# shrubb/latent-pose-reenactment

Hardware: AMD Instinct MI355X
Metric: train-step images/sec at 256x256 bs=8 (higher is better)
Workload: dtype mixed 16-bit MFMA operands, fp32 accumulate, fp32 activations / weights / optimizer state; 1 GPU; default.yaml meta-training step (configs[2]): ResNeXt50 identity encoder over 8 frames + MobileNetV2 pose encoder (both trained, forward + backward on hand-written gfx950 kernels), G, D with the 98000x512 label embedding, VGG19/VGGFace/featmat/adversarial/dis_embed/dice criterions, Adam, EMA; image_size=256, per_gpu_batch=8, global_batch=8, parallelism=dp1, precision_mode=default assignment (LP_PREC=f16), padding=zero, launch_mode=hipgraph

## Files before the change

### include/lp_hip.h

```cpp
#ifndef LP_HIP_H
#define LP_HIP_H
#include <stdint.h>
#ifdef __cplusplus
extern "C" {
#endif

#define LP_OK 0
#define LP_ERR_ARG (-1)
#define LP_ERR_UNSUPPORTED (-2)
#define LP_ERR_HIP (-3)

#define LP_PREC_BF16 0
#define LP_PREC_BF16X3 1
#define LP_PREC_F16 2

const char* lp_last_error(void);
int lp_abi_version(void);

int lp_pack_weights(const float* w, uint16_t* hi, uint16_t* lo, int Cout, int Cin, int T, int RowsP, int ColsP, int mode, int f16,
                    void* stream);
int lp_pack_desc_bytes(void);
int lp_pack_weights_batch(const void* table, int num_entries, long long total_chunks, void* stream);
int lp_pack_pair_desc_bytes(void);
int lp_pack_weights_pairs(const void* table, int num_entries, long long total_tiles, void* stream);

int lp_act_pack(const float* x, const float* scale, const float* shift, int pro, uint16_t* hi, uint16_t* lo,
                int N, int HW, int C, int prec, const float* in_scale, const float* amax_part, int amax_count, int amax_stride,
                float* scale_out, void* stream);
int lp_amax_blocks(void);
int lp_amax_slots(void);
int lp_amax_slot_stride(void);
int lp_amax_partial(const float* x, long long numel, float* part, void* stream);

int lp_conv16_fwd(const uint16_t* a_hi, const uint16_t* a_lo, const uint16_t* w_hi, const uint16_t* w_lo, float* y,
                  const float* bias, const float* res, const float* alpha, const float* alpha2,
                  int N, int H, int W, int Cin, int Cout, int CinP, int CoutP,
                  int ksize, int upsample, int res_shift, int prec, const uint16_t* relu_mask16,
                  uint16_t* out_hi, uint16_t* out_lo, int out_relu, float* workspace, long long workspace_bytes, float* amax_slots,
                  void* stream);
long long lp_conv16_fwd_workspace_bytes(int N, int H, int W, int Cout, int ksize);
int lp_conv16_fwd_stats(const uint16_t* a_hi, const uint16_t* a_lo, const uint16_t* w_hi, const uint16_t* w_lo, float* y,
                        const float* bias, const float* res, const float* alpha, const float* alpha2,
                        int N, int H, int W, int Cin, int Cout, int CinP, int CoutP,
                        int ksize, int upsample, int res_shift, int prec, const uint16_t* relu_mask16,
                        uint16_t* out_hi, uint16_t* out_lo, int out_relu, float* workspace, long long workspace_bytes, float* amax_slots,
                        float* stats, long long stats_capacity_floats, int* stats_rows, void* stream);
long long lp_conv16_stats_floats(int N, int H, int W, int Cout);
int lp_norm_stats_finalize(const float* part, int S, const float* gamma, const float* beta, int ab_stride, float eps, float momentum,
                           float* running_mean, float* running_var, float* mean, float* rstd, float* scale, float* shift,
                           int N, int C, void* stream);

long long lp_conv_wgrad_workspace_bytes(int Cin, int Cout, int ksize, int splits);
int lp_conv16_wgrad(const uint16_t* a_hi, const uint16_t* a_lo, const uint16_t* dy_hi, const uint16_t* dy_lo, float* dw,
                    float* workspace, int N, int H, int W, int Cin, int Cout, int ksize, int upsample, int splits, int prec,
                    float* dbias, int dbias_accumulate, const float* out_scale, const float* sn_w_orig, float* sn_dot, void* stream);
int lp_conv_wgrad_dot_blocks(int Cin, int Cout, int ksize);

int lp_thin_conv_supported(int Cin, int Cout, int ksize, int W);
int lp_thin_conv_fwd(const float* x, const uint16_t* w_hi, const uint16_t* w_lo, float* y, const float* bias, const float* alpha,
                     int N, int H, int W, int Cin, int Cout, int CinP, int CoutP, int ksize, int prec, uint16_t* out_hi, int out_relu,
                     void* stream);
int lp_thin_conv_emits_planes(int Cin, int Cout, int ksize, int W, int prec);
int lp_thin_wgrad_supported(int Cin, int Cout, int ksize, int pro, int W);
int lp_thin_wgrad_has_dbias(int Cin, int Cout);
int lp_thin_wgrad(const float* x, const float* dy, float* dw, float* workspace, const float* scale, const float* shift,
                  int N, int H, int W, int Cin, int Cout, int ksize, int pro, int splits, float* dbias, void* stream);

int lp_linear_fwd(const float* x, const float* w, const float* bias, const float* alpha, float* y, int B, int N, int K, void* stream);
long long lp_linear_bwd_workspace_bytes(int B, int N, int K);
int lp_linear_bwd(const float* x, const float* w, const float* g, const float* alpha, float* dx, float* dw, float* db,
                  float* workspace, int B, int N, int K, void* stream);

int lp_grid_crop_fwd(const float* images, const float* boxes, float* out, int N, int C, int H, int W, int Ho, int Wo, void* stream);
int lp_grid_crop_bwd(const float* dout, const float* boxes, float* dimages, int N, int C, int H, int W, int Ho, int Wo, void* stream);

int lp_stem_conv_s2(const float* x, const float* w, float* y, int N, int H, int W, int Cout, void* stream);
int lp_dwconv3x3_fwd(const float* x, const float* w, const float* in_scale, const float* in_shift, float* y,
                     int N, int H, int W, int C, int stride, void* stream);
int lp_affine_res(const float* y, const float* scale, const float* shift, const float* res, float* x, uint16_t* hi, uint16_t* lo,
                  long long P, int C, int prec, void* stream);
int lp_affine_relu6_mean(const float* y, const float* scale, const float* shift, float* out, int N, int HW, int C, void* stream);
long long lp_bn_stats_workspace_bytes(long long P, int C);
int lp_pwconv_stat_rows(long long P, int K, int N);
int lp_pwconv_fwd(const float* x, const float* w, float* y, const float* in_scale, const float* in_shift, int in_relu6,
                  const float* in_res, float* x_out, float* stats_part, long long P, int K, int N, void* stream);
int lp_dwconv_stat_rows(int N, int H, int W, int C, int stride);
int lp_dwconv3x3_stats_fwd(const float* x, const float* w, const float* in_scale, const float* in_shift, float* y, float* stats_part,
                           int N, int H, int W, int C, int stride, void* stream);
int lp_bn_finalize(const float* stats_part, int rows, const float* gamma, const float* beta, float* running_mean, float* running_var,
                   float* scale, float* shift, int C, float eps, float momentum, void* stream);
int lp_bn_stats(const float* y, const float* gamma, const float* beta, float* running_mean, float* running_var, float* scale,
                float* shift, float* workspace, long long P, int C, float eps, float momentum, void* stream);

// ... 163 lines not shown
```

### latent_pose_reenactment_amd/_lib.py

```python
import ctypes
import os

import torch

_HERE = os.path.dirname(os.path.abspath(__file__))
LIB_PATH = os.environ.get('LP_LIB_OVERRIDE') or os.path.join(_HERE, 'liblp_hip.so')

PREC_BF16 = 0
PREC_BF16X3 = 1
PREC_F16 = 2

_vp, _i, _f, _ll = ctypes.c_void_p, ctypes.c_int, ctypes.c_float, ctypes.c_longlong

SIGNATURES = {
    'lp_last_error': (ctypes.c_char_p, []),
    'lp_abi_version': (_i, []),
    'lp_pack_weights': (_i, [_vp, _vp, _vp, _i, _i, _i, _i, _i, _i, _i, _vp]),
    'lp_pack_desc_bytes': (_i, []),
    'lp_pack_weights_batch': (_i, [_vp, _i, _ll, _vp]),
    'lp_pack_pair_desc_bytes': (_i, []),
    'lp_pack_weights_pairs': (_i, [_vp, _i, _ll, _vp]),
    'lp_act_pack': (_i, [_vp, _vp, _vp, _i, _vp, _vp, _i, _i, _i, _i, _vp, _vp, _i, _i, _vp, _vp]),
    'lp_amax_slots': (_i, []),
    'lp_amax_slot_stride': (_i, []),
    'lp_amax_blocks': (_i, []),
    'lp_amax_partial': (_i, [_vp, _ll, _vp, _vp]),
    'lp_conv16_fwd': (_i, [_vp] * 9 + [_i] * 11 + [_vp, _vp, _vp, _i, _vp, _ll, _vp, _vp]),
    'lp_conv16_fwd_workspace_bytes': (_ll, [_i] * 5),
    'lp_conv16_fwd_stats': (_i, [_vp] * 9 + [_i] * 11 + [_vp, _vp, _vp, _i, _vp, _ll, _vp, _vp, _ll, _vp, _vp]),
    'lp_conv16_stats_floats': (_ll, [_i] * 4),
    'lp_norm_stats_finalize': (_i, [_vp, _i, _vp, _vp, _i, _f, _f, _vp, _vp, _vp, _vp, _vp, _vp, _i, _i, _vp]),
    'lp_gconv16_fwd_stats': (_i, [_vp] * 6 + [_i] * 6 + [_vp, _vp, _ll, _vp, _vp]),
    'lp_gconv16_fwd_planes': (_i, [_vp] * 8 + [_i] * 7 + [_vp, _vp, _ll, _vp, _vp]),
    'lp_conv_wgrad_workspace_bytes': (_ll, [_i, _i, _i, _i]),
    'lp_conv16_wgrad': (_i, [_vp] * 6 + [_i] * 9 + [_vp, _i, _vp, _vp, _vp, _vp]),
    'lp_conv_wgrad_dot_blocks': (_i, [_i] * 3),
    'lp_thin_conv_supported': (_i, [_i] * 4),
    'lp_thin_conv_fwd': (_i, [_vp] * 6 + [_i] * 9 + [_vp, _i, _vp]),
    'lp_thin_conv_emits_planes': (_i, [_i] * 5),
    'lp_thin_wgrad_supported': (_i, [_i] * 5),
    'lp_thin_wgrad_has_dbias': (_i, [_i] * 2),
    'lp_thin_wgrad': (_i, [_vp] * 6 + [_i] * 8 + [_vp, _vp]),
    'lp_linear_fwd': (_i, [_vp, _vp, _vp, _vp, _vp, _i, _i, _i, _vp]),
    'lp_linear_bwd_workspace_bytes': (_ll, [_i, _i, _i]),
    'lp_linear_bwd': (_i, [_vp] * 8 + [_i, _i, _i, _vp]),
    'lp_grid_crop_fwd': (_i, [_vp, _vp, _vp, _i, _i, _i, _i, _i, _i, _vp]),
    'lp_grid_crop_bwd': (_i, [_vp, _vp, _vp, _i, _i, _i, _i, _i, _i, _vp]),
    'lp_stem_conv_s2': (_i, [_vp, _vp, _vp, _i, _i, _i, _i, _vp]),
    'lp_dwconv3x3_fwd': (_i, [_vp] * 5 + [_i] * 5 + [_vp]),
    'lp_affine_res': (_i, [_vp] * 7 + [_ll, _i, _i, _vp]),
    'lp_affine_relu6_mean': (_i, [_vp] * 4 + [_i, _i, _i, _vp]),
    'lp_bn_stats_workspace_bytes': (_ll, [_ll, _i]),
    'lp_pwconv_stat_rows': (_i, [_ll, _i, _i]),
    'lp_pwconv_fwd': (_i, [_vp] * 5 + [_i, _vp, _vp, _vp, _ll, _i, _i, _vp]),
    'lp_dwconv_stat_rows': (_i, [_i] * 5),
    'lp_dwconv3x3_stats_fwd': (_i, [_vp] * 6 + [_i] * 5 + [_vp]),
    'lp_bn_finalize': (_i, [_vp, _i, _vp, _vp, _vp, _vp, _vp, _vp, _i, _f, _f, _vp]),
    'lp_bn_stats': (_i, [_vp] * 8 + [_ll, _i, _f, _f, _vp]),
    'lp_instnorm_workspace_bytes': (_ll, [_i, _i, _i]),
    'lp_instnorm_stats': (_i, [_vp, _vp, _vp, _i, _f, _vp, _vp, _vp, _vp, _vp, _i, _i, _i, _vp]),
    'lp_adain_bwd_workspace_bytes': (_ll, [_i, _i, _i]),
    'lp_adain_relu_bwd': (_i, [_vp, _vp, _vp, _vp, _i, _vp, _vp, _vp, _vp, _vp, _vp, _vp, _vp, _i, _i, _i, _i, _i, _vp, _vp]),
    'lp_norm_act_bwd': (_i, [_vp, _vp, _vp, _vp, _i, _vp, _vp, _vp, _vp, _vp, _vp, _vp, _vp, _i, _i, _i, _i, _i, _i, _vp, _vp, _f, _i, _vp, _vp]),
    'lp_bn_train_stats_workspace_bytes': (_ll, [_ll, _i]),
    'lp_bn_train_stats': (_i, [_vp, _vp, _vp, _f, _f, _vp, _vp, _vp, _vp, _vp, _vp, _vp, _ll, _i, _vp]),
    'lp_gconv16_fwd': (_i, [_vp] * 6 + [_i] * 6 + [_vp, _vp]),
    'lp_gconv_wgrad_workspace_bytes': (_ll, [_i, _i]),
    'lp_gconv16_wgrad': (_i, [_vp] * 6 + [_i] * 7 + [_vp, _vp]),
    'lp_pack_grouped': (_i, [_vp, _vp, _vp, _i, _i, _i, _i, _i, _vp]),
    'lp_im2col_planes': (_i, [_vp, _vp, _vp] + [_i] * 8 + [_vp]),
    'lp_bn_relu_maxpool_fwd': (_i, [_vp] * 7 + [_i] * 5 + [_vp]),
    'lp_maxpool_bwd': (_i, [_vp, _vp, _vp, _i, _i, _i, _i, _vp]),
    'lp_bn_add_act': (_i, [_vp] * 9 + [_ll, _i, _i, _i, _vp]),
    'lp_bn_add_act_planes': (_i, [_vp] * 8 + [_ll, _i, _i, _i, _vp]),
    'lp_bn_add_act16': (_i, [_vp] * 8 + [_ll, _i, _i, _vp]),
    'lp_bn_act16': (_i, [_vp] * 4 + [_ll, _i, _i, _vp]),
    'lp_adain_act16': (_i, [_vp] * 4 + [_i, _ll, _i, _i, _vp]),
    'lp_adain_relu_bwd16': (_i, [_vp, _vp, _vp, _vp, _i, _vp, _vp, _vp, _vp, _vp, _vp, _vp, _vp, _i, _i, _i, _i, _i, _vp, _vp]),
    'lp_thin_wgrad16': (_i, [_vp] * 6 + [_i] * 8 + [_vp]),
    'lp_subsample2': (_i, [_vp, _vp, _i, _i, _i, _i, _vp]),
    'lp_zero_stuff2': (_i, [_vp, _vp, _i, _i, _i, _i, _vp]),
# ... 87 lines not shown
```

### latent_pose_reenactment_amd/build.py

```python
import os
import subprocess
import sys
import time
from concurrent.futures import ThreadPoolExecutor

HERE = os.path.dirname(os.path.abspath(__file__))
CSRC = os.path.join(HERE, 'csrc')
INCLUDE = os.path.join(os.path.dirname(HERE), 'include')
LIB = os.path.join(HERE, 'liblp_hip.so')
SOURCES = ['lp_api.hip', 'elementwise.hip', 'tanh_head.hip', 'spectral_norm.hip', 'act_pack.hip', 'conv_dma.hip', 'conv_pipe.hip', 'conv_wgrad.hip', 'conv_thin.hip', 'conv_stem8.hip', 'linear_crop.hip', 'mobilenet.hip', 'resnext.hip', 'reflect_border.hip', 'stickman.hip']
FLAGS = ['--offload-arch=gfx950', '-O3', '-std=c++17', '-fPIC', '-I', INCLUDE, '-I', CSRC]


def _newer(a, b):
    return not os.path.exists(b) or os.path.getmtime(a) > os.path.getmtime(b)


def build(force: bool = False, verbose: bool = True) -> str:
    hipcc = os.environ.get('HIPCC', '/opt/rocm/bin/hipcc')
    objdir = os.path.join(HERE, 'build')
    os.makedirs(objdir, exist_ok=True)
    headers = [os.path.join(CSRC, f) for f in os.listdir(CSRC) if f.endswith('.h')] + [os.path.join(INCLUDE, 'lp_hip.h')]
    jobs = []
    for src in SOURCES:
        s = os.path.join(CSRC, src)
        o = os.path.join(objdir, src.replace('.hip', '.o'))
        if force or _newer(s, o) or any(_newer(h, o) for h in headers):
            jobs.append((s, o))

    def compile_one(job):
        s, o = job
        t_start = time.time()
        cmd = [hipcc] + FLAGS + ['-c', s, '-o', o]
        if verbose:
            print('[lp build]', ' '.join(cmd), flush=True)
        r = subprocess.run(cmd, capture_output=True, text=True)
        if r.returncode != 0:
            raise RuntimeError(f'hipcc failed for {s}:\n{r.stderr}')
        os.utime(o, (t_start, t_start))
        return o

    with ThreadPoolExecutor(max_workers=4) as ex:
        list(ex.map(compile_one, jobs))
    objs = [os.path.join(objdir, s.replace('.hip', '.o')) for s in SOURCES]
    if jobs or not os.path.exists(LIB):
        cmd = [hipcc, '--offload-arch=gfx950', '-shared', '-fPIC', '-o', LIB] + objs
        if verbose:
            print('[lp build]', ' '.join(cmd), flush=True)
        r = subprocess.run(cmd, capture_output=True, text=True)
        if r.returncode != 0:
            raise RuntimeError(f'link failed:\n{r.stderr}')
    return LIB


if __name__ == '__main__':
    print(build(force='--force' in sys.argv))
```

### latent_pose_reenactment_amd/csrc/conv_common.h

```cpp
#pragma once
#include "lp_common.h"
#include <stdlib.h>

struct Conv16Params {
    const uint16_t* a_hi; const uint16_t* a_lo; const uint16_t* w_hi; const uint16_t* w_lo;
    float* y;
    const float* bias; const float* res; const float* alpha; const float* alpha2;
    const uint16_t* mask16;
    uint16_t* o_hi; uint16_t* o_lo;
    int o_relu;
    float* amax;
    float* part; long long part_bytes;
    int N, H, W, Hin, Win, Cin, C8, Cout, Co8, CinP, CoutP;
    int res_shift;
    int lTH, lTW, lNB, tiles_x, tiles_y;
    int hit;
    int a_dbuf;
    int ksplit;
    float* stats;
    long long stats_cap;
    int stats_rows;
    int xcd_map, ntiles, nco;
    int phase;
    int grouped;
};

static inline int ilog2_floor(int v) { int l = 0; while ((1 << (l + 1)) <= v) ++l; return l; }

__device__ __forceinline__ bool conv16_block(const Conv16Params& p, int& tile, int& cob) {
    if (!p.xcd_map) { tile = (int)blockIdx.x; cob = (int)blockIdx.y; return true; }
    const int id = (int)blockIdx.x, x = id & 7, j = id >> 3;
    if (p.xcd_map == 2) { tile = id % p.ntiles; cob = id / p.ntiles; return cob < p.nco; }
    const int per = (p.ntiles + 7) >> 3;
    cob = j % p.nco;
    const int k = j / p.nco;
    tile = x * per + k;
    return k < per && tile < p.ntiles;
}

static inline dim3 conv16_grid(Conv16Params& p, int ntiles, int nco, int gz = 1) {
    static const int on = getenv("LP_CONV_XCD") ? atoi(getenv("LP_CONV_XCD")) : 1;
    p.ntiles = ntiles; p.nco = nco;
    p.xcd_map = (on && nco > 1 && ntiles >= 16) ? on : 0;
    if (!p.xcd_map) return dim3(ntiles, nco, gz);
    return dim3(((ntiles + 7) / 8) * 8 * nco, 1, gz);
}

static inline void choose_tile(int BM, int N, int H, int W, int* lTH, int* lTW, int* lNB) {
    int lbm = ilog2_floor(BM);
    int ltw = ilog2_floor(W); if (ltw > 4) ltw = 4;
    int lth = ilog2_floor(H); if (lth > lbm - ltw) lth = lbm - ltw;
    if (lth < 1) lth = 1;
    if (ltw < 1) ltw = 1;
    int lnb = lbm - ltw - lth; if (lnb < 0) lnb = 0;
    while (lnb > 0 && (1 << (lnb - 1)) >= N) --lnb;
    *lTH = lth; *lTW = ltw; *lNB = lnb;
}

int lp_conv_pipe_launch(Conv16Params& p, int ups, int prec, hipStream_t s);
int lp_conv1x1_pipe_launch(Conv16Params& p, int prec, hipStream_t s);

template <int WM, int WN, int MR, int NR, int PREC, int MRP>
__device__ __forceinline__ void conv16_epilogue(const Conv16Params& p, f32x4_t (&acc)[MR][NR], unsigned char* smem, int wave_d, int wm, int wn,
                                                int lane, int n0, int y0, int x0, int co0, int NBv, int tile_index, int ph = -1) {
    constexpr bool SPLIT = (PREC == LP_PREC_BF16X3), F16 = (PREC == LP_PREC_F16);
    float alpha = p.alpha ? *p.alpha : 1.f;
    if (p.alpha2) alpha *= *p.alpha2;
    if ((p.Cout & 3) == 0) {
        constexpr int WR = MR * 16, WC = NR * 16, LDW = WC + 4;
        __syncthreads();
        float* tile = (float*)smem + wave_d * (MRP * 16 * LDW);
        constexpr int C4 = WC / 4;
        constexpr int RPP = 64 / C4;
        const int c4 = lane % C4, rsub = lane / C4;
        const int co = co0 + wn * WC + c4 * 4;
        float4 bv = make_float4(0.f, 0.f, 0.f, 0.f);
        if (p.bias && co < p.Cout) bv = *(const float4*)(p.bias + co);
        float am = 0.f;
        float st_n = 0.f, st_ref[4] = {0.f, 0.f, 0.f, 0.f}, st_d[4] = {0.f, 0.f, 0.f, 0.f}, st_q[4] = {0.f, 0.f, 0.f, 0.f};
#pragma unroll
        for (int mp = 0; mp < MR; mp += MRP) {
#pragma unroll
            for (int mr = mp; mr < mp + MRP; ++mr)
#pragma unroll
                for (int nr = 0; nr < NR; ++nr)
#pragma unroll
                    for (int r = 0; r < 4; ++r)
                        tile[((mr - mp) * 16 + (lane >> 4) * 4 + r) * LDW + nr * 16 + (lane & 15)] = acc[mr][nr][r];
#pragma unroll 4
        for (int r0 = mp * 16; r0 < (mp + MRP) * 16; r0 += RPP) {
            const int row = r0 + rsub;
            const int m = wm * WR + row;
            int nb, py, px;
            tile_row_linear(m, p.lTH, p.lTW, nb, py, px);
            const int n = n0 + nb;
            int oyy = y0 + py, oxx = x0 + px;
            bool inside = nb < NBv && n < p.N && co < p.Cout;
            if (ph >= 0) { inside = inside && oyy < p.Hin && oxx < p.Win; oyy = 2 * oyy + (ph >> 1); oxx = 2 * oxx + (ph & 1); }
            else inside = inside && oyy < p.H && oxx < p.W;
            if (inside) {
                float4 v = *(const float4*)(tile + (row - mp * 16) * LDW + c4 * 4);
                if (p.ksplit > 1) {
                    const size_t pixs = (size_t)(n * p.H + oyy) * p.W + oxx;
                    *(float4*)(p.part + ((size_t)blockIdx.z * p.N * p.H * p.W + pixs) * p.Cout + co) = v;
                    continue;
                }
                v.x = fmaf(v.x, alpha, bv.x); v.y = fmaf(v.y, alpha, bv.y); v.z = fmaf(v.z, alpha, bv.z); v.w = fmaf(v.w, alpha, bv.w);
                if (p.res) {
                    const float4 rv = *(const float4*)(p.res + ((size_t)(n * (p.H >> p.res_shift) + (oyy >> p.res_shift)) * (p.W >> p.res_shift)
                                                                + (oxx >> p.res_shift)) * p.Cout + co);
                    v.x += rv.x; v.y += rv.y; v.z += rv.z; v.w += rv.w;
                }
                const size_t pix = (size_t)(n * p.H + oyy) * p.W + oxx;
// ... 98 lines not shown
```

### latent_pose_reenactment_amd/csrc/conv_dma.hip

```cpp
#include "lp_common.h"
#include "conv_common.h"
#include "lp_hip.h"
#include "lp_internal.h"
#include <stdlib.h>
#include <type_traits>

__device__ __attribute__((aligned(64))) unsigned int lp_zero_page[16];


template <int KS, bool UPS, int WM, int WN, int MR, int NR, int PREC, bool PP, int NBUF = 2, int CC = 32, bool GH = false>
#ifndef LP_PP_MINW
#define LP_PP_MINW 2
#endif
#ifndef LP_X3_1X1_MINW
#define LP_X3_1X1_MINW 3
#endif
__global__ __launch_bounds__(WM * WN * 64 * (PP ? 2 : 1), (PP && PREC != LP_PREC_BF16X3) ? LP_PP_MINW : (!PP && NBUF == 2 && WM * WN == 4 && PREC != LP_PREC_BF16X3) ? 2 :
                             (KS == 1 && !PP && WM * WN == 4 && PREC == LP_PREC_BF16X3) ? LP_X3_1X1_MINW : 1)
void conv_dma_kernel(Conv16Params p) {
    constexpr int ROWB = CC * 2;
    constexpr int SL = CC / 8, RPI = 64 / SL;
    constexpr int KK = CC / 32;
    static_assert(CC == 32 || CC == 64, "32- or 64-channel chunks");
    constexpr bool SPLIT = (PREC == LP_PREC_BF16X3), F16 = (PREC == LP_PREC_F16);
// ... 367 lines not shown
    const int tiles = p.tiles_x * p.tiles_y * ((p.N + NBv - 1) / NBv) * (phf ? 4 : 1);
    constexpr bool pp_ok = (KS == 3 || KS == 2) && (NWAVE == 4);
    static const int pp_env = getenv("LP_CONV_PP") ? atoi(getenv("LP_CONV_PP")) : -1;
    const long long pp_wgs = (long long)((tiles + 1) / 2) * ((p.Cout + BN - 1) / BN);
    const bool pp = pp_ok && (pp_env >= 0 ? pp_env != 0 : pp_wgs >= 200) && tiles >= 2 && p.a_dbuf && (!phf || ((p.tiles_x * p.tiles_y) & 1) == 0);
    if (pp) epi *= 2;
    if (lds < epi) lds = epi;
    if (lds > LDS_MAX) return lp_set_error(LP_ERR_UNSUPPORTED, "conv16 tile needs too much LDS");
    dim3 grid(pp ? (tiles + 1) / 2 : tiles, (p.Cout + BN - 1) / BN);
    p.xcd_map = 0; p.ntiles = grid.x; p.nco = grid.y;
    {
        static const int max_split = getenv("LP_CONV_KSPLIT") ? atoi(getenv("LP_CONV_KSPLIT")) : 8;
        static const int split_wgs = getenv("LP_CONV_SPLIT_WGS") ? atoi(getenv("LP_CONV_SPLIT_WGS")) : 256;
        const int wgs = grid.x * grid.y, nch = (p.CinP / CC) * (phd ? 4 : 1);
        int ks = 1;
        if ((KS == 3 || KS == 2) && (p.Cout & 3) == 0 && p.part)
            while (ks < max_split && wgs * ks * 2 <= split_wgs && nch / (ks * 2) >= 2 &&
                   (long long)(ks * 2) * p.N * p.H * p.W * p.Cout * (long long)sizeof(float) <= p.part_bytes) ks *= 2;
        for (;;) { const int per = (nch + ks - 1) / ks, k2 = (nch + per - 1) / per; if (k2 == ks) break; ks = k2; }
        p.ksplit = ks;
        grid.z = ks;
    }
    if ((KS == 3 || KS == 2) && !p.grouped) grid = conv16_grid(p, (int)grid.x, (int)grid.y, (int)grid.z);
    p.stats_rows = 0;
    if (p.stats) {
        constexpr int WR = MR * 16;
        const long long rows = (long long)(pp ? 2 * ((tiles + 1) / 2) : tiles) * WM;
        const bool ok = (NBv * TH * TW == BM) && (TH * TW >= WR) && (GHt % TH == 0) && (GWt % TW == 0) && ((p.Cout & 3) == 0) && p.ksplit == 1 &&
                        rows * p.Cout * 3 <= p.stats_cap && (!phf || NBv == 1);
        if (ok) p.stats_rows = (p.H * p.W) / WR; else p.stats = nullptr;
    }
    if constexpr (pp_ok) { if (pp) return launch_v<KS, UPS, WM, WN, MR, NR, PREC, true, 2, CC, GH>(p, lds, grid, stream); }
    if constexpr (KS == 1 && CC == 32 && !GH) { if (b1) return launch_v<KS, UPS, WM, WN, MR, NR, PREC, false, 1, CC, GH>(p, lds, grid, stream); }
    constexpr int NQ = KS * BN * ROWB / 1024;
    constexpr bool ring_ok = (NQ % NWAVE == 0);
    static const int nbuf_env = getenv("LP_CONV_NBUF") ? atoi(getenv("LP_CONV_NBUF")) : 0;
    if constexpr (ring_ok) {
        const size_t lds3 = lds_halo + 3 * B_BUF;
        const long long total_wgs = (long long)grid.x * grid.y * grid.z;
        const bool ring = (nbuf_env ? nbuf_env == 3 : total_wgs <= 320) && lds3 <= LDS_MAX;
        if (ring) return launch_v<KS, UPS, WM, WN, MR, NR, PREC, false, 3, CC, GH>(p, lds3 > epi ? lds3 : epi, grid, stream);
    }
    return launch_v<KS, UPS, WM, WN, MR, NR, PREC, false, 2, CC, GH>(p, lds, grid, stream);
}

template <int PREC>
static int dispatch_conv16(Conv16Params& p, int ks, int ups, hipStream_t s) {
    if (ks == 3 && ups >= 2) {
        const int gh = ups == 2 ? p.Hin : p.H, gw = ups == 2 ? p.Win : p.W;
        if ((p.Cout & 3) || gh < 2 || gw < 2) return lp_set_error(LP_ERR_UNSUPPORTED, "phase-decomposed conv: Cout % 4 == 0, low-resolution grid >= 2 x 2");
        if (p.Cout <= 64 && gh * gw >= 256) return launch_conv16<2, false, 4, 1, 4, 4, PREC>(p, s);
        return launch_conv16<2, false, 2, 2, 4, 4, PREC>(p, s);
    }
    if (ks == 3) {
        const int r = lp_conv_pipe_launch(p, ups, PREC, s);
        if (r) return r < 0 ? r : LP_OK;
    }
    if (ks == 1 && !ups) {
        const int r = lp_conv1x1_pipe_launch(p, PREC, s);
        if (r) return r < 0 ? r : LP_OK;
    }
    const bool big_img = p.H * p.W >= 256;
    static const int w8_env = getenv("LP_CONV_W8") ? atoi(getenv("LP_CONV_W8")) : -1;
    const bool w8 = w8_env >= 0 ? (w8_env != 0) : (p.H * p.W <= 256);
    if (w8 && p.Cout > 64) {
        static const int x3bn64 = getenv("LP_CONV_X3_BN64") ? atoi(getenv("LP_CONV_X3_BN64")) : 1;
        if (PREC == LP_PREC_BF16X3 && x3bn64 && ks == 3) {
            if (!ups) return launch_conv16<3, false, 2, 2, 4, 2, PREC>(p, s);
            return launch_conv16<3, true, 2, 2, 4, 2, PREC>(p, s);
        }
        if (ks == 3 && !ups) return launch_conv16<3, false, 2, 4, 4, 2, PREC>(p, s);
        if (ks == 3 && ups) return launch_conv16<3, true, 2, 4, 4, 2, PREC>(p, s);
        if (ks == 1 && !ups) return launch_conv16<1, false, 2, 4, 4, 2, PREC>(p, s);
    }
    if (PREC == LP_PREC_BF16X3 && ks == 3 && p.Cout > 64) {
        static const int x3mid = getenv("LP_CONV_X3_BN64") ? atoi(getenv("LP_CONV_X3_BN64")) : 1;
        const long long tiles128 = ((long long)p.N * p.H * p.W + 127) / 128;
        if (x3mid >= 2 && ((tiles128 + 1) / 2) * ((p.Cout + 127) / 128) < 200) {
            if (!ups) return launch_conv16<3, false, 2, 2, 4, 2, PREC>(p, s);
            return launch_conv16<3, true, 2, 2, 4, 2, PREC>(p, s);
        }
    }
    if (ks == 3 && !ups) {
        if (p.Cout <= 16 && big_img) return launch_conv16<3, false, 4, 1, 4, 1, PREC>(p, s);
        if (p.Cout <= 64 && big_img) return launch_conv16<3, false, 4, 1, 4, 4, PREC>(p, s);
        return launch_conv16<3, false, 2, 2, 4, 4, PREC>(p, s);
    }
    if (ks == 3 && ups) {
        if (p.Cout <= 64 && big_img) return launch_conv16<3, true, 4, 1, 4, 4, PREC>(p, s);
        return launch_conv16<3, true, 2, 2, 4, 4, PREC>(p, s);
    }
    if (ks == 1 && !ups) {
        static const int cc_env = getenv("LP_CONV_CC1") ? atoi(getenv("LP_CONV_CC1")) : 0;
        const bool cc64 = (cc_env ? cc_env == 64 : (p.Cin >= 512 && PREC != LP_PREC_BF16X3)) && (p.CinP % 64 == 0);
        static const int tile_env = getenv("LP_CONV1X1_TILE") ? atoi(getenv("LP_CONV1X1_TILE")) : 0;
        const long long pix = (long long)p.N * p.H * p.W;
        const bool tall = (tile_env ? tile_env == 256 : false) && p.Cout >= 128 && p.H * p.W >= 256 &&
                          (pix / 256) * ((p.Cout + 127) / 128) >= 512;
        if (cc64) {
            if (p.Cout <= 64 && big_img) return launch_conv16<1, false, 4, 1, 4, 4, PREC, 64>(p, s);
            if (tall) return launch_conv16<1, false, 4, 2, 4, 4, PREC, 64>(p, s);
            return launch_conv16<1, false, 2, 2, 4, 4, PREC, 64>(p, s);
        }
        if (p.Cout <= 64 && big_img) return launch_conv16<1, false, 4, 1, 4, 4, PREC>(p, s);
        if (tall) return launch_conv16<1, false, 4, 2, 4, 4, PREC>(p, s);
        return launch_conv16<1, false, 2, 2, 4, 4, PREC>(p, s);
    }
    return lp_set_error(LP_ERR_UNSUPPORTED, "unsupported conv configuration");
}

extern "C" long long lp_conv16_fwd_workspace_bytes(int N, int H, int W, int Cout, int ksize) {
    if (ksize != 3 || (Cout & 3)) return 0;
    const long long P = (long long)N * H * W;
    const long long wgs_lb = ((P + 255) / 256) * ((Cout + 127) / 128);
    static const int max_split = getenv("LP_CONV_KSPLIT") ? atoi(getenv("LP_CONV_KSPLIT")) : 8;
    static const int split_wgs = getenv("LP_CONV_SPLIT_WGS") ? atoi(getenv("LP_CONV_SPLIT_WGS")) : 256;
    long long ks = split_wgs / wgs_lb; if (ks > max_split) ks = max_split;
    if (ks < 2) return 0;
    return ks * P * Cout * (long long)sizeof(float);
}

extern "C" int lp_conv16_fwd(const uint16_t* a_hi, const uint16_t* a_lo, const uint16_t* w_hi, const uint16_t* w_lo, float* y,
                             const float* bias, const float* res, const float* alpha, const float* alpha2,
                             int N, int H, int W, int Cin, int Cout, int CinP, int CoutP,
                             int ksize, int upsample, int res_shift, int prec, const uint16_t* relu_mask16,
                             uint16_t* out_hi, uint16_t* out_lo, int out_relu, float* workspace, long long workspace_bytes, float* amax_slots,
                             void* stream) {
    if (!y) return lp_set_error(LP_ERR_ARG, "lp_conv16_fwd: null pointer");
    return lp_conv16_fwd_stats(a_hi, a_lo, w_hi, w_lo, y, bias, res, alpha, alpha2, N, H, W, Cin, Cout, CinP, CoutP, ksize, upsample, res_shift, prec,
                               relu_mask16, out_hi, out_lo, out_relu, workspace, workspace_bytes, amax_slots, nullptr, 0, nullptr, stream);
}

extern "C" int lp_conv16_fwd_stats(const uint16_t* a_hi, const uint16_t* a_lo, const uint16_t* w_hi, const uint16_t* w_lo, float* y,
                                   const float* bias, const float* res, const float* alpha, const float* alpha2,
                                   int N, int H, int W, int Cin, int Cout, int CinP, int CoutP,
                                   int ksize, int upsample, int res_shift, int prec, const uint16_t* relu_mask16,
                                   uint16_t* out_hi, uint16_t* out_lo, int out_relu, float* workspace, long long workspace_bytes, float* amax_slots,
                                   float* stats, long long stats_capacity_floats, int* stats_rows, void* stream) {
    if (stats_rows) *stats_rows = 0;
    if (!a_hi || !w_hi) return lp_set_error(LP_ERR_ARG, "lp_conv16_fwd: null pointer");
    if (!y && (!out_hi || (Cout & 7))) return lp_set_error(LP_ERR_ARG, "lp_conv16_fwd: y may only be NULL when out_hi is given and Cout % 8 == 0");
    if (stats && !stats_rows) return lp_set_error(LP_ERR_ARG, "lp_conv16_fwd: stats needs stats_rows");
    if (prec == LP_PREC_BF16X3 && (!w_lo || !a_lo)) return lp_set_error(LP_ERR_ARG, "lp_conv16_fwd: bf16x3 needs the lo planes");
    if (prec == LP_PREC_BF16X3 && out_hi && !out_lo) return lp_set_error(LP_ERR_ARG, "lp_conv16_fwd: bf16x3 needs out_lo");
    if ((upsample == 1 || upsample == 2) && ((H | W) & 1)) return lp_set_error(LP_ERR_ARG, "lp_conv16_fwd: upsampled output dims must be even");
    if (upsample < 0 || upsample > 3) return lp_set_error(LP_ERR_ARG, "lp_conv16_fwd: upsample = 0 | 1 | 2 (phase form) | 3 (phase form of the data gradient)");
    if (CinP % 32 || CinP < Cin || CoutP % 128 || CoutP < Cout) return lp_set_error(LP_ERR_ARG, "lp_conv16_fwd: bad padded dims");
    if (H < 2 || W < 2) return lp_set_error(LP_ERR_UNSUPPORTED, "lp_conv16_fwd: H,W must be >= 2");
    Conv16Params p;
    p.a_hi = a_hi; p.a_lo = a_lo; p.w_hi = w_hi; p.w_lo = w_lo; p.y = y; p.bias = bias; p.res = res; p.alpha = alpha; p.alpha2 = alpha2;
    p.mask16 = relu_mask16; p.o_relu = out_relu; p.part = workspace; p.part_bytes = workspace ? workspace_bytes : 0; p.amax = amax_slots;
    p.o_hi = (Cout & 7) ? nullptr : out_hi; p.o_lo = (Cout & 7) ? nullptr : out_lo;
    p.N = N; p.H = H; p.W = W; p.Hin = upsample ? H / 2 : H; p.Win = upsample ? W / 2 : W;
    p.Cin = Cin; p.C8 = (Cin + 7) & ~7; p.Cout = Cout; p.Co8 = (Cout + 7) & ~7; p.CinP = CinP; p.CoutP = CoutP; p.res_shift = res_shift;
    p.grouped = 0; p.stats = stats; p.stats_cap = stats ? stats_capacity_floats : 0; p.stats_rows = 0;
    p.phase = (upsample == 2) ? 1 : (upsample == 3) ? 2 : 0;
    if (upsample >= 2 && ksize != 3) return lp_set_error(LP_ERR_ARG, "lp_conv16_fwd: upsample = 2 | 3 (phase-decomposed forms) are 3x3 forms");
    if (upsample == 3) { p.Hin = 2 * H; p.Win = 2 * W; }
    hipStream_t s = (hipStream_t)stream;
    int rc;
    if (prec == LP_PREC_BF16) rc = dispatch_conv16<LP_PREC_BF16>(p, ksize, upsample, s);
    else if (prec == LP_PREC_BF16X3) rc = dispatch_conv16<LP_PREC_BF16X3>(p, ksize, upsample, s);
    else if (prec == LP_PREC_F16) rc = dispatch_conv16<LP_PREC_F16>(p, ksize, upsample, s);
    else return lp_set_error(LP_ERR_ARG, "lp_conv16_fwd: unknown precision mode");
    if (rc) return rc;
// ... 61 lines not shown
```

Before: 201.5 images/s.

## Add whole-K-in-LDS small-spatial conv kernel with split-K for tiny feature maps

```diff
diff --git a/include/lp_hip.h b/include/lp_hip.h
--- a/include/lp_hip.h
+++ b/include/lp_hip.h
@@ -39,6 +39,7 @@
                   uint16_t* out_hi, uint16_t* out_lo, int out_relu, float* workspace, long long workspace_bytes, float* amax_slots,
                   void* stream);
 long long lp_conv16_fwd_workspace_bytes(int N, int H, int W, int Cout, int ksize);
+long long lp_conv_small_launches(void);
 int lp_conv16_fwd_stats(const uint16_t* a_hi, const uint16_t* a_lo, const uint16_t* w_hi, const uint16_t* w_lo, float* y,
                         const float* bias, const float* res, const float* alpha, const float* alpha2,
                         int N, int H, int W, int Cin, int Cout, int CinP, int CoutP,
diff --git a/latent_pose_reenactment_amd/_lib.py b/latent_pose_reenactment_amd/_lib.py
--- a/latent_pose_reenactment_amd/_lib.py
+++ b/latent_pose_reenactment_amd/_lib.py
@@ -27,6 +27,7 @@
     'lp_amax_partial': (_i, [_vp, _ll, _vp, _vp]),
     'lp_conv16_fwd': (_i, [_vp] * 9 + [_i] * 11 + [_vp, _vp, _vp, _i, _vp, _ll, _vp, _vp]),
     'lp_conv16_fwd_workspace_bytes': (_ll, [_i] * 5),
+    'lp_conv_small_launches': (_ll, []),
     'lp_conv16_fwd_stats': (_i, [_vp] * 9 + [_i] * 11 + [_vp, _vp, _vp, _i, _vp, _ll, _vp, _vp, _ll, _vp, _vp]),
     'lp_conv16_stats_floats': (_ll, [_i] * 4),
     'lp_norm_stats_finalize': (_i, [_vp, _i, _vp, _vp, _i, _f, _f, _vp, _vp, _vp, _vp, _vp, _vp, _i, _i, _vp]),
diff --git a/latent_pose_reenactment_amd/build.py b/latent_pose_reenactment_amd/build.py
--- a/latent_pose_reenactment_amd/build.py
+++ b/latent_pose_reenactment_amd/build.py
@@ -8,7 +8,7 @@
 CSRC = os.path.join(HERE, 'csrc')
 INCLUDE = os.path.join(os.path.dirname(HERE), 'include')
 LIB = os.path.join(HERE, 'liblp_hip.so')
-SOURCES = ['lp_api.hip', 'elementwise.hip', 'tanh_head.hip', 'spectral_norm.hip', 'act_pack.hip', 'conv_dma.hip', 'conv_pipe.hip', 'conv_wgrad.hip', 'conv_thin.hip', 'conv_stem8.hip', 'linear_crop.hip', 'mobilenet.hip', 'resnext.hip', 'reflect_border.hip', 'stickman.hip']
+SOURCES = ['lp_api.hip', 'elementwise.hip', 'tanh_head.hip', 'spectral_norm.hip', 'act_pack.hip', 'conv_dma.hip', 'conv_small.hip', 'conv_pipe.hip', 'conv_wgrad.hip', 'conv_thin.hip', 'conv_stem8.hip', 'linear_crop.hip', 'mobilenet.hip', 'resnext.hip', 'reflect_border.hip', 'stickman.hip']
 FLAGS = ['--offload-arch=gfx950', '-O3', '-std=c++17', '-fPIC', '-I', INCLUDE, '-I', CSRC]
 
 
diff --git a/latent_pose_reenactment_amd/csrc/conv_common.h b/latent_pose_reenactment_amd/csrc/conv_common.h
--- a/latent_pose_reenactment_amd/csrc/conv_common.h
+++ b/latent_pose_reenactment_amd/csrc/conv_common.h
@@ -59,6 +59,8 @@
 
 int lp_conv_pipe_launch(Conv16Params& p, int ups, int prec, hipStream_t s);
 int lp_conv1x1_pipe_launch(Conv16Params& p, int prec, hipStream_t s);
+int lp_conv_small_launch(Conv16Params& p, int ksize, int ups, int prec, hipStream_t s);
+long long lp_conv_small_workspace_bytes(int N, int H, int W, int Cout, int ksize);
 
 template <int WM, int WN, int MR, int NR, int PREC, int MRP>
 __device__ __forceinline__ void conv16_epilogue(const Conv16Params& p, f32x4_t (&acc)[MR][NR], unsigned char* smem, int wave_d, int wm, int wn,
diff --git a/latent_pose_reenactment_amd/csrc/conv_dma.hip b/latent_pose_reenactment_amd/csrc/conv_dma.hip
--- a/latent_pose_reenactment_amd/csrc/conv_dma.hip
+++ b/latent_pose_reenactment_amd/csrc/conv_dma.hip
@@ -443,6 +443,10 @@
         if (p.Cout <= 64 && gh * gw >= 256) return launch_conv16<2, false, 4, 1, 4, 4, PREC>(p, s);
         return launch_conv16<2, false, 2, 2, 4, 4, PREC>(p, s);
     }
+    {
+        const int r = lp_conv_small_launch(p, ks, ups, PREC, s);
+        if (r) return r < 0 ? r : LP_OK;
+    }
     if (ks == 3) {
         const int r = lp_conv_pipe_launch(p, ups, PREC, s);
         if (r) return r < 0 ? r : LP_OK;
@@ -502,6 +506,8 @@
 
 extern "C" long long lp_conv16_fwd_workspace_bytes(int N, int H, int W, int Cout, int ksize) {
     if (ksize != 3 || (Cout & 3)) return 0;
+    const long long small = lp_conv_small_workspace_bytes(N, H, W, Cout, ksize);
+    if (small) return small;
     const long long P = (long long)N * H * W;
     const long long wgs_lb = ((P + 255) / 256) * ((Cout + 127) / 128);
     static const int max_split = getenv("LP_CONV_KSPLIT") ? atoi(getenv("LP_CONV_KSPLIT")) : 8;
diff --git a/latent_pose_reenactment_amd/csrc/conv_small.hip b/latent_pose_reenactment_amd/csrc/conv_small.hip
--- /dev/null
+++ b/latent_pose_reenactment_amd/csrc/conv_small.hip
@@ -0,0 +1,291 @@
+#include "lp_common.h"
+#include "conv_common.h"
+#include "lp_hip.h"
+#include "lp_internal.h"
+#include <atomic>
+
+static __device__ __attribute__((aligned(64))) unsigned int lp_zero_page_small[16];
+
+static std::atomic<long long> small_launches{0};
+extern "C" long long lp_conv_small_launches(void) { return small_launches.load(std::memory_order_relaxed); }
+
+#define LP_W1(n) case n: lp_wait_vm<n>(); break;
+#define LP_W4(n) LP_W1(n) LP_W1(n + 1) LP_W1(n + 2) LP_W1(n + 3)
+#define LP_W16(n) LP_W4(n) LP_W4(n + 4) LP_W4(n + 8) LP_W4(n + 12)
+__device__ __forceinline__ void wait_vm_uniform(int n) {
+    switch (n) {
+        LP_W16(0) LP_W16(16) LP_W16(32) LP_W16(48)
+        default: lp_wait_vm0(); break;
+    }
+}
+
+constexpr int SM_HMAX = 8;
+constexpr int SM_NW = 4;
+
+template <int KS, int WM, int WN, int MR, int NR, int PREC>
+__global__ __launch_bounds__(256, 1)
+void conv_small_kernel(Conv16Params p, int per) {
+    static_assert(WM * WN == SM_NW, "four waves");
+    constexpr bool SPLIT = (PREC == LP_PREC_BF16X3), F16 = (PREC == LP_PREC_F16);
+    constexpr int NPL = SPLIT ? 2 : 1;
+    constexpr int BN = WN * NR * 16;
+    constexpr int RW = KS * BN * 64 / 1024;
+    constexpr int W_BYTES = KS * RW * 1024;
+    constexpr int SG = (KS == 1) ? 4 : 1;
+    static_assert((KS * BN) % 16 == 0, "a kernel row is a whole number of DMA pieces");
+
+    extern __shared__ __attribute__((aligned(16))) unsigned char smem[];
+
+    const int tid = (int)threadIdx.x, lane = tid & 63;
+    const int wave = __builtin_amdgcn_readfirstlane(tid >> 6);
+    const int wm = wave / WN, wn = wave % WN;
+    const int TH = 1 << p.lTH, TW = 1 << p.lTW, NBv = 1 << p.lNB;
+
+    int t = (int)blockIdx.x;
+    const int tile_id = t, cob = (int)blockIdx.y;
+    const int tx = t % p.tiles_x; t /= p.tiles_x;
+    const int ty = t % p.tiles_y; t /= p.tiles_y;
+    const int n0 = t << p.lNB, y0 = ty << p.lTH, x0 = tx << p.lTW;
+    const int co0 = cob * BN;
+    const int HH = TH + KS - 1, HW = TW + KS - 1, oy = y0 - KS / 2, ox = x0 - KS / 2;
+    const int halo_px = NBv * HH * HW;
+    const int NH = p.hit;
+    const int a_bytes = NH * 1024;
+    const int ch_bytes = NPL * (a_bytes + W_BYTES);
+
+    const int nch_total = p.CinP / 32;
+    const int cbeg = (int)blockIdx.z * per;
+    const int nch = min(nch_total, cbeg + per) - cbeg;
+
+    auto rkey = [](int r) { return (r >> 1) & 3; };
+    const int wofs = (wave - NH) & 3;
+    auto mine = [&](int n) { return (n + SM_NW - 1 - wave) / SM_NW; };
+    auto minew = [&](int n) { return (n + SM_NW - 1 - wofs) / SM_NW; };
+    const int hcnt = mine(NH);
+
+    {
+        const int rr = lane >> 2, slot = lane & 3;
+        const int g8 = (slot ^ rkey(rr)) * 8;
+        int a_off[SM_HMAX];
+#pragma unroll
+        for (int k = 0; k < SM_HMAX; ++k) {
+            const int hp = (k * SM_NW + wave) * 16 + rr;
+            const int hx = hp % HW, t2 = hp / HW;
+            const int hy = t2 % HH, nb = t2 / HH;
+            const int n = n0 + nb, iy = oy + hy, ix = ox + hx;
+            const bool inb = (hp < halo_px) && (n < p.N) && (iy >= 0) && (iy < p.Hin) && (ix >= 0) && (ix < p.Win);
+            a_off[k] = inb ? (((n * p.Hin + iy) * p.Win + ix) * p.C8 + g8) : -1;
+        }
+        const uint16_t* zero16 = (const uint16_t*)lp_zero_page_small;
+        for (int c = 0; c < nch; ++c) {
+            const int c0 = (cbeg + c) * 32;
+            const bool cok = (c0 + g8) < p.C8;
+            const unsigned dst = (unsigned)__builtin_amdgcn_readfirstlane((int)(unsigned)(uintptr_t)(smem + c * ch_bytes));
+#pragma unroll
+            for (int k = 0; k < SM_HMAX; ++k) {
+                if (k < hcnt) {
+                    const bool ok = cok && a_off[k] >= 0;
+                    const size_t off = (size_t)(ok ? a_off[k] + c0 : 0);
+                    const unsigned d = dst + (unsigned)((k * SM_NW + wave) * 1024);
+                    lp_glds16(ok ? (p.a_hi + off) : zero16, d);
+                    if (SPLIT) lp_glds16(ok ? (p.a_lo + off) : zero16, d + a_bytes);
+                }
+            }
+            const unsigned dstw = dst + (unsigned)(NPL * a_bytes);
+#pragma unroll
+            for (int q0 = 0; q0 < KS * RW; q0 += SM_NW) {
+                const int q = q0 + wofs;
+                if ((KS * RW) % SM_NW == 0 || q < KS * RW) {
+                    const int r = q * 16 + rr;
+                    const int tap = r / BN, n = r % BN;
+                    const size_t off = ((size_t)(tap * p.CoutP + co0 + n) * p.CinP + c0 + g8);
+                    lp_glds16(p.w_hi + off, dstw + q * 1024);
+                    if (SPLIT) lp_glds16(p.w_lo + off, dstw + W_BYTES + q * 1024);
+                }
+            }
+        }
+    }
+
+    int a_nbbase[MR], a_py[MR], a_px[MR];
+#pragma unroll
+    for (int mr = 0; mr < MR; ++mr) {
+        const int m = wm * (MR * 16) + mr * 16 + (lane & 15);
+        int nb, py, px;
+        tile_row_linear(m, p.lTH, p.lTW, nb, py, px);
+        a_nbbase[mr] = nb * HH * HW; a_py[mr] = py; a_px[mr] = px;
+    }
+    const int kb = lane >> 4;
+    const int bsl = (kb ^ rkey(lane & 15)) << 4;
+    int b_off[NR];
+#pragma unroll
+    for (int nr = 0; nr < NR; ++nr) b_off[nr] = (wn * (NR * 16) + nr * 16 + (lane & 15)) * 64 + bsl;
+
+    f32x4_t acc[MR][NR];
+#pragma unroll
+    for (int mr = 0; mr < MR; ++mr)
+#pragma unroll
+        for (int nr = 0; nr < NR; ++nr) acc[mr][nr] = (f32x4_t){0.f, 0.f, 0.f, 0.f};
+
+    const int wcnt_all = minew(KS * RW);
+    const int pc = NPL * (hcnt + wcnt_all);
+    const int total = nch * pc;
+
+    for (int c = 0; c < nch; ++c) {
+        const unsigned char* A_hi = smem + c * ch_bytes;
+        const unsigned char* A_lo = A_hi + a_bytes;
+        const unsigned char* B_hi = A_hi + NPL * a_bytes;
+#pragma unroll
+        for (int ky = 0; ky < KS; ++ky) {
+            if (KS == 3 || (c % SG) == 0) {
+                const int cl = (KS == 3) ? c : min(c + SG - 1, nch - 1);
+                const int through = cl * pc + NPL * (hcnt + ((KS == 3) ? minew((ky + 1) * RW) : wcnt_all));
+                wait_vm_uniform(total - through);
+                __syncthreads();
+            }
+#pragma unroll
+            for (int kx = 0; kx < KS; ++kx) {
+                const unsigned char* Bk = B_hi + (ky * KS + kx) * (BN * 64);
+                s16x8_t fa[MR], fal[MR], fb[NR], fbl[NR];
+#pragma unroll
+                for (int mr = 0; mr < MR; ++mr) {
+                    const int hp = a_nbbase[mr] + (a_py[mr] + ky) * HW + a_px[mr] + kx;
+                    const int off = hp * 64 + ((kb ^ rkey(hp)) << 4);
+                    fa[mr] = *(const s16x8_t*)(A_hi + off);
+                    if (SPLIT) fal[mr] = *(const s16x8_t*)(A_lo + off);
+                }
+#pragma unroll
+                for (int nr = 0; nr < NR; ++nr) {
+                    fb[nr] = *(const s16x8_t*)(Bk + b_off[nr]);
+                    if (SPLIT) fbl[nr] = *(const s16x8_t*)(Bk + W_BYTES + b_off[nr]);
+                }
+#pragma unroll
+                for (int mr = 0; mr < MR; ++mr)
+#pragma unroll
+                    for (int nr = 0; nr < NR; ++nr) {
+                        if (SPLIT) {
+                            acc[mr][nr] = mfma16(fal[mr], fb[nr], acc[mr][nr]);
+                            acc[mr][nr] = mfma16(fa[mr], fbl[nr], acc[mr][nr]);
+                        }
+                        acc[mr][nr] = mfma16t<F16>(fa[mr], fb[nr], acc[mr][nr]);
+                    }
+            }
+        }
+    }
+
+    conv16_epilogue<WM, WN, MR, NR, PREC, MR>(p, acc, smem, wave, wm, wn, lane, n0, y0, x0, co0, NBv, tile_id);
+}
+
+constexpr size_t SM_LDS_MAX = 160 * 1024;
+constexpr int SM_VM_MAX = 60;
+constexpr int SM_KS_MAX = 16;
+
+struct SmallPlan { int per, ks, hit, lTH, lTW, lNB, tiles_x, tiles_y, tiles; size_t lds; };
+
+template <int KS>
+static bool small_plan(const Conv16Params& p, int BM, int BN, int planes, int ks_want, SmallPlan& o) {
+    choose_tile(BM, p.N, p.H, p.W, &o.lTH, &o.lTW, &o.lNB);
+    const int TH = 1 << o.lTH, TW = 1 << o.lTW, NBv = 1 << o.lNB;
+    if (NBv * TH * TW > BM) return false;
+    const int halo_px = NBv * (TH + KS - 1) * (TW + KS - 1);
+    o.hit = (halo_px + 15) / 16;
+    if ((o.hit + SM_NW - 1) / SM_NW > SM_HMAX) return false;
+    o.tiles_x = (p.W + TW - 1) / TW; o.tiles_y = (p.H + TH - 1) / TH;
+    o.tiles = o.tiles_x * o.tiles_y * ((p.N + NBv - 1) / NBv);
+    const int wq = KS * KS * BN * 64 / 1024;
+    const size_t chunk = (size_t)planes * (o.hit + wq) * 1024;
+    int pc = 0;
+    for (int w = 0; w < SM_NW; ++w) {
+        const int wofs = (w - o.hit) & 3, n = planes * ((o.hit + SM_NW - 1 - w) / SM_NW + (wq + SM_NW - 1 - wofs) / SM_NW);
+        if (n > pc) pc = n;
+    }
+    int fit = (int)(SM_LDS_MAX / chunk);
+    if (fit > SM_VM_MAX / pc) fit = SM_VM_MAX / pc;
+    if (fit < 1) return false;
+    const int nch = p.CinP / 32;
+    int ks = ks_want < 1 ? 1 : ks_want;
+    if (ks > nch) ks = nch;
+    int per = (nch + ks - 1) / ks;
+    if (per > fit) {
+        if (ks_want < 1) return false;
+        per = fit;
+    }
+    o.per = per; o.ks = (nch + per - 1) / per;
+    o.lds = chunk * per;
+    return true;
+}
+
+template <int KS, int WM, int WN, int MR, int NR, int PREC>
+static int launch_small(Conv16Params& p, const SmallPlan& pl, hipStream_t stream) {
+    auto kern = conv_small_kernel<KS, WM, WN, MR, NR, PREC>;
+    static thread_local int attr_dev = -1;
+    int dev = 0;
+    if (hipGetDevice(&dev) != hipSuccess) return lp_set_error(LP_ERR_HIP, "hipGetDevice failed");
+    if (attr_dev != dev) {
+        if (hipFuncSetAttribute((const void*)kern, hipFuncAttributeMaxDynamicSharedMemorySize, (int)SM_LDS_MAX) != hipSuccess)
+            return lp_set_error(LP_ERR_HIP, "hipFuncSetAttribute failed");
+        attr_dev = dev;
+    }
+    p.lTH = pl.lTH; p.lTW = pl.lTW; p.lNB = pl.lNB; p.tiles_x = pl.tiles_x; p.tiles_y = pl.tiles_y; p.hit = pl.hit;
+    p.a_dbuf = 0; p.ksplit = pl.ks; p.xcd_map = 0; p.ntiles = pl.tiles;
+    p.stats = nullptr; p.stats_rows = 0;
+    constexpr int BN = WN * NR * 16;
+    p.nco = (p.Cout + BN - 1) / BN;
+    size_t lds = pl.lds;
+    const size_t epi = (size_t)SM_NW * MR * 16 * (NR * 16 + 4) * sizeof(float);
+    if (lds < epi) lds = epi;
+    if (lds > SM_LDS_MAX) return lp_set_error(LP_ERR_UNSUPPORTED, "conv_small: tile needs too much LDS");
+    hipLaunchKernelGGL(kern, dim3(pl.tiles, p.nco, pl.ks), dim3(256), lds, stream, p, pl.per);
+    const int rc = lp_check_launch("conv_small");
+    if (rc) return rc;
+    small_launches.fetch_add(1, std::memory_order_relaxed);
+    return 1;
+}
+
+long long lp_conv_small_workspace_bytes(int N, int H, int W, int Cout, int ksize) {
+    static const int on = getenv("LP_CONV_SMALL") ? atoi(getenv("LP_CONV_SMALL")) : 1;
+    if (!on || ksize != 3 || (Cout & 3) || H > 8 || W > 8 || (long long)N * H * W > 512) return 0;
+    return (long long)SM_KS_MAX * N * H * W * Cout * (long long)sizeof(float);
+}
+
+template <int PREC>
+static int conv_small_dispatch(Conv16Params& p, int ks, hipStream_t s) {
+    constexpr int planes = (PREC == LP_PREC_BF16X3) ? 2 : 1;
+    const long long P = (long long)p.N * p.H * p.W;
+    const int nch = p.CinP / 32;
+    SmallPlan pl;
+    if (ks == 1) {
+        if (p.stats) return 0;
+        if (!small_plan<1>(p, 32, 32, planes, 0, pl)) return 0;
+        return launch_small<1, 2, 2, 1, 1, PREC>(p, pl, s);
+    }
+    if (p.stats && nch < 4) return 0;
+    const long long wbytes = 9LL * p.Cout * p.CinP * 2 * planes, slice = P * p.Cout * (long long)sizeof(float);
+    long long ks_cap = wbytes / slice;
+    if (ks_cap < 2) ks_cap = 2;
+    if (ks_cap > SM_KS_MAX) ks_cap = SM_KS_MAX;
+    const long long ks_ws = ((p.Cout & 3) || !p.part) ? 1 : p.part_bytes / slice;
+    if (ks_cap > ks_ws) ks_cap = ks_ws;
+    if (ks_cap < 1) ks_cap = 1;
+    static const int bn_env = getenv("LP_CONV_SMALL_BN") ? atoi(getenv("LP_CONV_SMALL_BN")) : 0;
+    const long long mt = (P + 127) / 128;
+    int bn = bn_env ? bn_env : (mt * ((p.Cout + 63) / 64) * ks_cap >= 256 ? 64 : 32);
+    for (int attempt = 0; attempt < 2; ++attempt, bn = (bn == 64 ? 32 : 64)) {
+        if (!small_plan<3>(p, 128, bn, planes, (int)ks_cap, pl)) continue;
+        if (pl.ks > ks_cap) continue;
+        const long long per_cu = (long long)(SM_LDS_MAX / (pl.lds < 20 * 1024 ? 20 * 1024 : pl.lds));
+        if ((long long)pl.tiles * ((p.Cout + bn - 1) / bn) * pl.ks > 256 * per_cu) continue;
+        if (bn == 64) return launch_small<3, 2, 2, 4, 2, PREC>(p, pl, s);
+        return launch_small<3, 4, 1, 2, 2, PREC>(p, pl, s);
+    }
+    return 0;
+}
+
+int lp_conv_small_launch(Conv16Params& p, int ksize, int ups, int prec, hipStream_t s) {
+    static const int on = getenv("LP_CONV_SMALL") ? atoi(getenv("LP_CONV_SMALL")) : 1;
+    if (!on || ups || p.grouped || p.phase || (ksize != 3 && ksize != 1)) return 0;
+    if (p.H > 8 || p.W > 8 || (long long)p.N * p.H * p.W > 512) return 0;
+    if (prec == LP_PREC_BF16) return conv_small_dispatch<LP_PREC_BF16>(p, ksize, s);
+    if (prec == LP_PREC_BF16X3) return conv_small_dispatch<LP_PREC_BF16X3>(p, ksize, s);
+    if (prec == LP_PREC_F16) return conv_small_dispatch<LP_PREC_F16>(p, ksize, s);
+    return 0;
+}
```

Result: slower. 198.4 images/s (-1.5%).
